# cliangyu/video-diffusion

Measured on AMD Instinct MI355X. Metric: denoise-steps/sec, higher is better.
Workload: dtype f32

## Files before the change

include/vd_amd.h:

```cpp
#ifndef VD_AMD_H
#define VD_AMD_H
#ifdef __cplusplus
extern "C" {
#endif

typedef struct vd_config {
    int image_size;
    int num_channels;
    int num_res_blocks;
    int num_heads;
    int T;
    int n_attention_ds;
    int attention_ds[8];
    int use_scale_shift_norm;
    int use_spatial_encoding;
    int use_frame_encoding;
    int enforce_position_invariance;
    int use_rpe_net;
    int allow_interactions_between_padding;
    float rp_alpha, rp_beta, rp_gamma;
    int time_embed_mult;
    int cond_emb_type;
    int learn_sigma;
} vd_config;
// ... 82 lines not shown
int vd_prior_bpd(vd_engine* e, int B, int T, const float* x_start, const float* latent_mask, float* out, void* stream);

int vd_score_windows(vd_engine* e, int B, int T, const float* x_start, const float* obs_mask, const float* latent_mask,
                     const float* kinda_marg_mask, const long long* frame_indices, const long long* t, int clip_denoised,
                     unsigned long long seed, const unsigned long long* item_offset, const float* noise, int suffix_skip,
                     double* mse_out, void* stream);
int vd_op_eps_mse(vd_engine* e, int B, int T, const float* x_start, const float* eps, const long long* t, int clip_denoised,
                  const float* latent_mask, unsigned long long seed, const unsigned long long* item_offset, const float* noise,
                  double* mse_out, void* stream);

int vd_window_begin(vd_engine* e, int B, int T, float* x, const float* obs_src, const float* obs_mask,
                    const float* latent_mask, const float* kinda_marg_mask, const long long* frame_indices,
                    int observed_frames, int sampler, int clip_denoised, float eta, unsigned long long seed,
                    unsigned long long offset, long long t_start, void* stream);
int vd_window_run(vd_engine* e, int n_steps, void* stream);
unsigned long long vd_window_generation(vd_engine* e);
int vd_window_graphs(vd_engine* e);

int vd_set_window_prefix_cache(vd_engine* e, int on);
int vd_window_prefix_frames(vd_engine* e);

int vd_set_window_suffix_skip(vd_engine* e, int on);
int vd_window_suffix_frames(vd_engine* e);

int vd_set_cfg_scale(vd_engine* e, float w);
float vd_cfg_scale(vd_engine* e);
int vd_op_cfg_combine(const float* out_c, const float* out_u, float w, long long n, float* out, void* stream);

int vd_set_guidance_rescale(vd_engine* e, float phi);
float vd_guidance_rescale(vd_engine* e);
int vd_set_dynamic_threshold(vd_engine* e, float p);
float vd_dynamic_threshold(vd_engine* e);
int vd_op_cfg_rescale(const float* out_c, const float* out_u, float w, const float* lat, int B, int T, long long frame_elems, float phi,
                      float* out, float* factor_out, void* stream);
int vd_op_dynamic_threshold(const float* x0, const float* lat, int B, int T, long long frame_elems, float p, float* out, float* s_out,
                            void* stream);

int vd_set_known_region(vd_engine* e, const float* known_src, const float* known_mask, const float* known_noise,
                        unsigned long long seed, unsigned long long offset);
int vd_known_region(vd_engine* e);
int vd_known_merge(vd_engine* e, int B, int T, long long frame_pixels, float* sample, const float* known_src, const float* known_mask,
                   const float* latent_mask, const long long* t, const float* known_noise, unsigned long long seed,
                   unsigned long long offset, void* stream);
int vd_set_jump_rows(vd_engine* e, int num_timesteps, const float* sqrt_alpha, const float* sqrt_beta);
int vd_q_jump(vd_engine* e, int B, int T, long long frame_pixels, const float* x, const float* latent_mask, const long long* t,
              const float* noise, unsigned long long seed, unsigned long long offset, float* out, void* stream);
// ... 157 lines not shown
```

video-diffusion_amd/_lib.py:

```python
import ctypes
import os
import subprocess

_HERE = os.path.dirname(os.path.abspath(__file__))
_CSRC = os.path.join(_HERE, "csrc")
SO_PATH = os.path.join(_HERE, "libvdamd.so")
SOURCES = ["igemm.hip", "conv_wino.hip", "conv_wino_r64.hip", "conv_wino_z128.hip", "gemm_frag.hip", "gemm_split.hip", "split_pack.hip", "norm.hip", "backward.hip", "attn_spatial.hip", "attn_temporal.hip", "attn_temporal_long.hip", "misc.hip", "guidance.hip", "known.hip", "measure.hip", "dps.hip", "engine.hip", "lpips.hip", "metrics.hip", "i3d.hip", "conv_cl.hip", "hallway.hip"]
HEADER = os.path.join(os.path.dirname(_HERE), "include", "vd_amd.h")
HEADERS = [os.path.join(_CSRC, "vd_common.h"), os.path.join(_CSRC, "wino_common.h"), os.path.join(_CSRC, "igemm_tile.h"), HEADER]
SOURCE_FLAGS = {"conv_wino_z128.hip": ["-mllvm", "-pragma-unroll-threshold=1000000"]}


def _toolchain():
    hipcc = os.environ.get("HIPCC", "/opt/rocm/bin/hipcc")
    flags = ["--offload-arch=gfx950", "-O3", "-std=c++17", "-fPIC", "-Wno-unused-value"] + \
        os.environ.get("VD_HIPCC_FLAGS", "").split()
    return hipcc, flags


def _sha(*parts):
    import hashlib
    h = hashlib.sha1()
    for p in parts:
        h.update(p if isinstance(p, bytes) else str(p).encode())
# ... 115 lines not shown
    "vd_pos_channels": (_I, [_P]),
    "vd_pos_resolution": (_I, [_P]),
    "vd_set_freqs": (_I, [_P, _P, _I, _P, _I]),
    "vd_set_schedule": (_I, [_P, _I, _P, _P, _F]),
    "vd_workspace_bytes": (_I, [_P, _I, _I, ctypes.POINTER(_L)]),
    "vd_unet_forward": (_I, [_P, _I, _I, _P, _P, _P, _P, _P, _P, _P, _I, _P, _P]),
    "vd_p_sample": (_I, [_P, _I, _I, _P, _P, _P, _P, _P, _P, _P, _I, _I, _P, _U, _U, _P, _P, _P, _P]),
    "vd_ddim_sample": (_I, [_P, _I, _I, _P, _P, _P, _P, _P, _P, _P, _I, _I, _F, _P, _U, _U, _P, _P, _P, _P]),
    "vd_ddim_reverse_sample": (_I, [_P, _I, _I, _P, _P, _P, _P, _P, _P, _P, _I, _I, _P, _P, _P, _P]),
    "vd_ddim_reverse_from_xstart": (_I, [_P, _I, _L, _P, _P, _P, _I, _P, _P, _P]),
    "vd_set_multistep_weights": (_I, [_P, _I, _P]),
    "vd_dpmpp_2m_sample": (_I, [_P, _I, _I, _P, _P, _P, _P, _P, _P, _P, _P, _I, _I, _P, _P, _P, _P]),
    "vd_dpmpp_2m_from_xstart": (_I, [_P, _I, _L, _P, _P, _P, _P, _I, _P, _P, _P]),
    "vd_p_mean_variance": (_I, [_P, _I, _I, _P, _P, _P, _P, _P, _P, _P, _I, _I, _P, _P, _P, _P]),
    "vd_vb_terms": (_I, [_P, _I, _I, _P, _P, _P, _P, _P, _I, _P, _P, _P, _P, _P, _P]),
    "vd_prior_bpd": (_I, [_P, _I, _I, _P, _P, _P, _P]),
    "vd_score_windows": (_I, [_P, _I, _I, _P, _P, _P, _P, _P, _P, _I, _U, _P, _P, _I, _P, _P]),
    "vd_op_eps_mse": (_I, [_P, _I, _I, _P, _P, _P, _I, _P, _U, _P, _P, _P, _P]),
    "vd_window_generation": (_U, [_P]),
    "vd_set_window_prefix_cache": (_I, [_P, _I]),
    "vd_window_prefix_frames": (_I, [_P]),
    "vd_set_window_suffix_skip": (_I, [_P, _I]),
    "vd_window_suffix_frames": (_I, [_P]),
    "vd_set_cfg_scale": (_I, [_P, _F]),
    "vd_cfg_scale": (_F, [_P]),
    "vd_op_cfg_combine": (_I, [_P, _P, _F, _L, _P, _P]),
    "vd_set_guidance_rescale": (_I, [_P, _F]),
    "vd_guidance_rescale": (_F, [_P]),
    "vd_set_dynamic_threshold": (_I, [_P, _F]),
    "vd_dynamic_threshold": (_F, [_P]),
    "vd_op_cfg_rescale": (_I, [_P, _P, _F, _P, _I, _I, _L, _F, _P, _P, _P]),
    "vd_op_dynamic_threshold": (_I, [_P, _P, _I, _I, _L, _F, _P, _P, _P]),
    "vd_set_known_region": (_I, [_P, _P, _P, _P, _U, _U]),
    "vd_known_region": (_I, [_P]),
    "vd_known_merge": (_I, [_P, _I, _I, _L, _P, _P, _P, _P, _P, _P, _U, _U, _P]),
    "vd_set_jump_rows": (_I, [_P, _I, _P, _P]),
    "vd_q_jump": (_I, [_P, _I, _I, _L, _P, _P, _P, _P, _U, _U, _P, _P]),
    "vd_window_jump": (_I, [_P, _I, _P]),
    "vd_set_measurement": (_I, [_P, _P, _I, _I]),
    "vd_measurement": (_I, [_P, _P, _P]),
    "vd_measurement_project": (_I, [_P, _I, _I, _I, _I, _P, _P, _P, _I, _I, _P]),
    "vd_window_begin": (_I, [_P, _I, _I, _P, _P, _P, _P, _P, _P, _I, _I, _I, _F, _U, _U, _L, _P]),
    "vd_window_run": (_I, [_P, _I, _P]),
    "vd_window_graphs": (_I, [_P]),
    "vd_posterior_update": (_I, [_P, _I, _I, _L, _P, _P, _P, _I, _F, _P, _U, _U, _P, _P, _P]),
    "vd_posterior_from_xstart": (_I, [_P, _I, _I, _L, _P, _P, _P, _I, _F, _P, _U, _U, _P, _P, _P, _P]),
# ... 71 lines not shown
    "vd_i3d_load_weight": (_I, [_P, ctypes.c_char_p, _P, _L]),
    "vd_i3d_max_frames": (_I, []),
    "vd_i3d_embed": (_I, [_P, _I, _I, _I, _I, _P, _P, _P]),
    "vd_op_conv3d_same": (_I, [_P, _P, _P, _I, _I, _I, _I, _I, _I, _I, _I, _I, _I, _I, _I, _P, _L, _P]),
    "vd_op_maxpool3d_same": (_I, [_P, _I, _I, _I, _I, _I, _I, _I, _I, _I, _I, _P, _P]),
    "vd_op_resize_bilinear_tf1": (_I, [_P, _I, _I, _I, _P, _P]),
    "vd_hallway_counts": (_I, [_I, _I, _I, _I, _I, _P, _I, _P, _P]),
    "vd_hallway_max_strip": (_I, []),
    "vd_op_green_mask": (_I, [_L, _P, _P, _P, _P]),
}

_lib = None


def lib():
    global _lib
    if _lib is None:
        path = os.environ.get("VD_LIB")
        if not path:
            build()
            path = SO_PATH
        L = ctypes.CDLL(path)
        for name, (res, args) in SIGNATURES.items():
            fn = getattr(L, name)
            fn.restype = res
            fn.argtypes = args
        if not os.environ.get("VD_LIB") and L.vd_source_sha().decode() != source_sha():
            raise RuntimeError(f"libvdamd.so was built from other sources ({L.vd_source_sha().decode()}) than the ones beside it "
                               f"({source_sha()}): rebuild (video_diffusion_amd._lib.build(force=True))")
        _lib = L
    return _lib


class VdError(RuntimeError):
    pass


def check(rc):
    if rc != 0:
        msg = lib().vd_last_error().decode(errors="replace")
        raise VdError(f"libvdamd error {rc}: {msg}")


def ptr(t):
    if t is None:
        return None
# ... 9 lines not shown
```

video-diffusion_amd/csrc/engine.hip:

```cpp
#include <cmath>
#include <cstring>
#include <unordered_map>
#include <vector>

#include "../../include/vd_amd.h"
#include "vd_common.h"

namespace vd {

thread_local std::string g_last_error;
void set_error(const std::string& msg) { g_last_error = msg; }

int launch_frame_t(const int64_t* fidx, int B, int T, int center, float* tv, hipStream_t s);

enum ParamKind { PK_RAW = 0, PK_CONV3, PK_STEM, PK_POSENC, PK_OUTCONV, PK_LINF, PK_CONV3W, PK_CONV3S,
                 PK_CONV3WU };

struct Param {
    std::string name;
    int nd = 0;
    long long shape[4] = {1, 1, 1, 1};
    size_t numel = 0;
    size_t packed = 0;
    size_t off = 0;
// ... 168 lines not shown
    std::vector<Param> params;
    std::unordered_map<std::string, int> pidx;
    std::vector<ResP> res;
    std::vector<AttnP> attn;
    std::vector<ConvP> convs;
    std::vector<std::vector<Layer>> input_blocks, output_blocks;
    std::vector<Layer> middle;
    int n_before_attn = 0, pos_res = 0, pos_ch = 0, final_ch = 0;
    int suf_blk = -2, suf_layer = -1;
    int p_posenc = -1, p_te0w, p_te0b, p_te2w, p_te2b, p_outgw, p_outgb, p_outw, p_outb;
    size_t film_w_off = 0, film_b_off = 0, te_w_off = 0, te_b_off = 0;
    int film_total = 0, te_total = 0;
    size_t packed_total = 0;
    float* wbuf = nullptr;
    bool wbuf_on_host = false;
    int put(void* dst, const void* src, size_t bytes) {
        if (wbuf_on_host) { std::memcpy(dst, src, bytes); return 0; }
        VD_HIP(hipMemcpy(dst, src, bytes, hipMemcpyHostToDevice));
        return 0;
    }
    struct RpeGroup { int C; std::vector<int> blocks; long long* d_hid = nullptr; long long* d_out = nullptr; };
    std::vector<RpeGroup> rpe_groups;
    std::vector<float*> rpe_R;
    int rpe_all(const float* te, const int64_t* fidx, int B, int T, hipStream_t st, Arena& ar);
    int rpe_tables();
    void rpe_group_blocks();
    float* d_freq_time = nullptr; int n_freq_time = 0;
    float* d_freq_frame = nullptr; int n_freq_frame = 0;
    float* d_tab = nullptr; int num_timesteps = 0;
    float* d_tmap = nullptr; float rescale = 1.f;
    float* d_w2m = nullptr;
    float* d_jump = nullptr;
    char* ws = nullptr; size_t ws_cap = 0;
    bool ws_suf = false;
    int ws_B = 0, ws_T = 0; size_t ws_tail = 0;
    std::unordered_map<long long, size_t> ws_peaks;
    static size_t tm_bytes(int B) { return ((size_t)B * sizeof(float) + 255) & ~(size_t)255; }
    size_t out_floats(int B, int T) const { return (size_t)B * T * (cfg.learn_sigma ? 6 : 3) * cfg.image_size * cfg.image_size; }
    size_t guid_off(int B, int T) const { return (tm_bytes(B) + 2 * out_floats(B, T) * sizeof(float) + 255) & ~(size_t)255; }
    size_t step_tail_bytes(int B, int T) const { return guid_off(B, T) + guidance_scratch_bytes(B); }
    float* step_tm() const { return reinterpret_cast<float*>(ws + ws_tail); }
    float* step_eps(int B) const { return reinterpret_cast<float*>(ws + ws_tail + tm_bytes(B)); }
    float* step_eps_u(int B, int T) const { return step_eps(B) + out_floats(B, T); }
    void* step_guid(int B, int T) const { return ws + ws_tail + guid_off(B, T); }
    Arena step_arena() const { Arena a; a.base = ws; a.cap = ws_tail; return a; }
    float* wbuf_bwd = nullptr; bool wbuf_bwd_on_host = false; size_t packed_bwd_total = 0;
    Tape* tape = nullptr;
// ... 73 lines not shown
        (void)hipDeviceSynchronize();
        for (auto& g : win_graphs) g.release();
        win_graphs.clear();
        win_cur = -1;
    }
    template <class Tp> int grow(Tp*& p, size_t& cap, size_t n, bool held_by_graphs) {
        if (n <= cap) return 0;
        if (held_by_graphs && p) { if (win_cur >= 0) win_lost = true; drop_window_graphs(); }
        if (p) VD_HIP(hipFree(p));
        p = nullptr; cap = 0;
        VD_HIP(hipMalloc(reinterpret_cast<void**>(&p), n * sizeof(Tp)));
        cap = n;
        return 0;
    }
    template <class DryRun> int grow_ws(long long key, size_t extra, DryRun dry_run, size_t* tail) {
        if (int rc = rpe_tables()) return rc;
        auto it = ws_peaks.find(key);
        if (it == ws_peaks.end()) {
            size_t peak = 0;
            if (int rc = dry_run(&peak)) return rc;
            it = ws_peaks.emplace(key, peak).first;
        }
        *tail = (it->second + 255) & ~(size_t)255;
        return grow(ws, ws_cap, *tail + extra, true);
    }

    const float* W(int p) const { return wbuf + params[p].off; }
    void set_w(vd::IgemmArgs& g, int p) const {
        const int k = params[p].kind;
        g.w = g.wfrag = g.wwino = nullptr;
        if (k == PK_CONV3W) { g.wwino = W(p); g.wsplit = split_math() ? 2 : 0; }
        else if (k == PK_CONV3WU) { g.wwino = W(p); g.wsplit = 2; g.ups_phase = 1; }
        else if (k == PK_CONV3S) { g.wfrag = W(p); g.wsplit = 1; }
        else if (k == PK_LINF) { g.wfrag = W(p); g.wsplit = split_math(); }
        else g.w = W(p);
    }

    int add(const std::string& name, std::initializer_list<long long> shape, int kind = PK_RAW) {
        Param p;
        p.name = name;
        p.nd = (int)shape.size();
        int i = 0;
        p.numel = 1;
        for (long long s : shape) { p.shape[i++] = s; p.numel *= (size_t)s; }
        p.kind = kind;
        p.packed = p.numel;
        const size_t O = (size_t)p.shape[0];
// ... 518 lines not shown
    if (!cfg.use_rpe_net || attn.empty() || !te_total) return 0;
    rpe_group_blocks();
    for (auto& g : rpe_groups) {
        if (g.d_hid) continue;
        const int nn = 3 * (int)g.blocks.size();
        std::vector<long long> th(3 * nn), to(2 * nn);
        for (size_t i = 0; i < g.blocks.size(); ++i) {
            const AttnP& a = attn[g.blocks[i]];
            const RpeP* rp[3] = {&a.rq, &a.rk, &a.rv};
            for (int k = 0; k < 3; ++k) {
                const int z = 3 * (int)i + k;
                th[3 * z] = rp[k]->te_off; th[3 * z + 1] = (long long)params[rp[k]->dw].off; th[3 * z + 2] = (long long)params[rp[k]->db].off;
                to[2 * z] = (long long)params[rp[k]->ow].off; to[2 * z + 1] = (long long)params[rp[k]->ob].off;
            }
        }
        VD_HIP(hipMalloc(reinterpret_cast<void**>(&g.d_hid), th.size() * sizeof(long long)));
        VD_HIP(hipMalloc(reinterpret_cast<void**>(&g.d_out), to.size() * sizeof(long long)));
        VD_HIP(hipMemcpy(g.d_hid, th.data(), th.size() * sizeof(long long), hipMemcpyHostToDevice));
        VD_HIP(hipMemcpy(g.d_out, to.data(), to.size() * sizeof(long long), hipMemcpyHostToDevice));
    }
    return 0;
}

int vd_engine::rpe_all(const float* te, const int64_t* fidx, int B, int T, hipStream_t st, Arena& ar) {
    rpe_R.clear();
    if (!cfg.use_rpe_net || attn.empty() || !te_total) return 0;
    rpe_group_blocks();
    const size_t rrows = (size_t)B * T * T;
    rpe_R.assign(3 * attn.size(), nullptr);
    int rc = 0;
    for (auto& g : rpe_groups) {
        const int nn = 3 * (int)g.blocks.size(), C = g.C;
        float* Rg = ar.get<float>((size_t)nn * rrows * C);
        for (size_t i = 0; i < g.blocks.size(); ++i)
            for (int k = 0; k < 3; ++k) rpe_R[3 * g.blocks[i] + k] = Rg + (3 * i + k) * rrows * C;
        const size_t mk = ar.mark();
        float* Eh = ar.get<float>((size_t)nn * rrows * C);
        ar.release(mk);
        if (ar.dry) continue;
        VD_REQUIRE(g.d_hid && g.d_out, "rpe_all: offset tables missing (ensure_ws builds them)");
        if ((rc = launch_rpe_hidden_tab(te, te_total, wbuf, g.d_hid, fidx, B, T, C, Eh, nn, rrows * C, st))) return rc;
        IgemmArgs q = linear_args((int)rrows, C, C);
        q.src0 = Eh; q.out = Rg;
        q.wfrag = wbuf + params[attn[g.blocks[0]].rq.ow].off; q.bias = wbuf + params[attn[g.blocks[0]].rq.ob].off;
        q.zcount = nn; q.zs_a = q.zs_out = (int)(rrows * C); q.ztab = g.d_out; q.zbase = wbuf;
        if ((rc = igemm_p(q, st))) return rc;
    }
    return 0;
}

int vd_engine::forward(const FwdIn& in, hipStream_t st, Arena& ar, const PrefixPlan* pp, const SuffixPlan* sp) {
    const int B = in.B, T = in.T, N = B * T, S = cfg.image_size, mc = cfg.num_channels;
    int rc;
    VD_REQUIRE(!pp || (!tape && !ar.dry && pp->store && n_before_attn > 0), "prefix plan: executor steps only");
    VD_REQUIRE(!sp || (!tape && sp->n > 0 && sp->n <= N && (ar.dry || sp->list)), "suffix plan: executor steps only, at least one frame");
    struct SelGuard { ~SelGuard() { g_sel_nfr = 0; } } sel_guard;
    const int Npre = pp ? pp->n : N;
    float* x8 = ar.get<float>((size_t)Npre * S * S * STEM_KPAD);
    float* tfr = ar.get<float>(N);
    float* amask = ar.get<float>(N);
    float* tsin = ar.get<float>((size_t)N * mc);
    float* e1 = ar.get<float>((size_t)N * E);
    float* emb = ar.get<float>((size_t)N * E);
    float* film = ar.get<float>((size_t)N * film_total);
    float* te = te_total ? ar.get<float>((size_t)N * te_total) : nullptr;
    float* ftv = cfg.use_frame_encoding ? ar.get<float>(N) : nullptr;
    float* femb = cfg.use_frame_encoding ? ar.get<float>((size_t)N * pos_ch) : nullptr;
    if (!ar.dry) {
        VD_REQUIRE(d_freq_time && n_freq_time == mc / 2, "vd_set_freqs not called (time frequencies)");
        AssembleArgs aa{in.x, in.obs_src, in.obs, in.lat, in.km, in.t_model, in.obs_mode, B, T, S, S, STEM_KPAD, cfg.cond_emb_type, x8, tfr, amask};
        if (pp) {
            AssembleArgs sc = aa; sc.scalars_only = 1;
            if ((rc = launch_assemble(sc, st))) return rc;
            aa.frame_list = pp->list; aa.n_list = pp->n;
        }
        if ((rc = launch_assemble(aa, st))) return rc;
        if ((rc = launch_sinus_embed(tfr, N, mc, d_freq_time, tsin, st))) return rc;
        if ((rc = linear(tsin, N, mc, E, W(p_te0w), W(p_te0b), 0, nullptr, e1, st))) return rc;
        if ((rc = linear(e1, N, E, E, W(p_te2w), W(p_te2b), 1, nullptr, emb, st))) return rc;
        if ((rc = linear(emb, N, E, film_total, wbuf + film_w_off, wbuf + film_b_off, 1, nullptr, film, st))) return rc;
        if (te_total && (rc = linear(emb, N, E, te_total, wbuf + te_w_off, wbuf + te_b_off, 0, nullptr, te, st))) return rc;
        if (cfg.use_frame_encoding) {
            VD_REQUIRE(d_freq_frame && n_freq_frame == pos_ch / 2, "vd_set_freqs not called (frame frequencies)");
            if ((rc = launch_frame_t(in.fidx, B, T, cfg.enforce_position_invariance, ftv, st))) return rc;
            if ((rc = launch_sinus_embed(ftv, N, pos_ch, d_freq_frame, femb, st))) return rc;
        }
    }
    rpe_R.clear();
    if (!(pp && pp->build_only) && (rc = rpe_all(te, in.fidx, B, T, st, ar))) return rc;
    attn_seq = 0;
    std::vector<Tens> hs;
    Tens h{x8, STEM_KPAD, S};
    int Nrun = Npre;
    const float* film_full = film;
    if (pp || ar.dry) {
        float* fc = ar.get<float>((size_t)std::max(pp ? Npre : N, 1) * film_total);
        if (pp) {
            if ((rc = launch_gather_rows(film_full, pp->list, Npre, film_total, fc, st))) return rc;
            film = fc;
        }
    }
    auto run = [&](const std::vector<Layer>& blk, Tens in0, const Tens* in1, Tens* outp, size_t l0 = 0, size_t l1 = ~(size_t)0) -> int {
        const int N = Nrun;
        Tens cur = in0;
        const Tens* second = in1;
        for (size_t li = l0; li < std::min(l1, blk.size()); ++li) {
            const Layer& L = blk[li];
            Tens nxt{};
            if (L.type == 1) {
                if ((rc = res_block(res[L.idx], cur, second, N, film, st, ar, &nxt))) return rc;
            } else if (L.type == 2) {
                if ((rc = attn_block(attn[L.idx], cur, B, T, in.fidx, amask, st, ar, &nxt))) return rc;
// ... 1162 lines not shown

int vd_op_dynamic_threshold(const float* x0, const float* lat, int B, int T, long long frame_elems, float p, float* out, float* s_out,
                            void* stream) {
    VD_REQUIRE(B > 0 && frame_elems > 0, "vd_op_dynamic_threshold: shape");
    OpScratch ws(stream);
    char* buf = nullptr;
    int rc = ws.get(&buf, guidance_scratch_bytes(B));
    if (rc) return rc;
    DynThreshArgs da{x0, nullptr, nullptr, nullptr, 0, lat, B, T, (long)frame_elems, p, out, s_out, nullptr, buf};
    return launch_dynamic_threshold(da, ws.st);
}

int vd_window_prefix_frames(vd_engine* e) {
    VD_REQUIRE(e, "null engine");
    return e->win_cur >= 0 && e->win_graphs[e->win_cur].store ? e->win_graphs[e->win_cur].n_inv : 0;
}

int vd_set_window_suffix_skip(vd_engine* e, int on) {
    VD_REQUIRE(e, "null engine");
    e->suffix_skip_on = on != 0;
    return 0;
}

int vd_window_suffix_frames(vd_engine* e) {
    VD_REQUIRE(e, "null engine");
    return e->win_cur >= 0 ? e->win_graphs[e->win_cur].n_suf : 0;
}

unsigned long long vd_window_generation(vd_engine* e) { return e ? e->win_gen : 0; }

int vd_window_run(vd_engine* e, int n_steps, void* stream) {
    VD_REQUIRE(e, "null engine");
    VD_REQUIRE(!e->win_lost, "window graphs invalidated (workspace growth or a new schedule since vd_window_begin): begin the window again");
    VD_REQUIRE(e->win_cur >= 0, "vd_window_begin first");
    const char* past = sampler_walks_up(e->win_graphs[e->win_cur].key.sampler) ? "more steps than the window has left (ddim_reverse_sample: t would pass num_timesteps - 1)"
                                                                  : "more steps than the window has left (t would pass 0)";
    VD_REQUIRE(n_steps >= 0 && n_steps <= e->win_left, past);
    hipStream_t st = static_cast<hipStream_t>(stream);
    for (int i = 0; i < n_steps; ++i) VD_HIP(hipGraphLaunch(e->win_graphs[e->win_cur].exec, st));
    e->win_left -= n_steps;
    return 0;
}

int vd_window_graphs(vd_engine* e) { return e ? (int)e->win_graphs.size() : -1; }

int vd_set_known_region(vd_engine* e, const float* known_src, const float* known_mask, const float* known_noise, unsigned long long seed,
// ... 688 lines not shown
```

video-diffusion_amd/csrc/gemm_split.hip:

```cpp
#include <cstring>
#include <vector>

#include "vd_common.h"

namespace vd {

typedef __bf16 bf16x4 __attribute__((ext_vector_type(4)));
typedef __bf16 bf16x8 __attribute__((ext_vector_type(8)));
typedef unsigned u32x4 __attribute__((ext_vector_type(4)));
typedef unsigned u32x2 __attribute__((ext_vector_type(2)));

template <bool F16>
__device__ __forceinline__ f32x16 mfma_piece(u32x4 a, u32x4 b, f32x16 c) {
    if constexpr (F16) return __builtin_amdgcn_mfma_f32_32x32x16_f16(__builtin_bit_cast(f16x8, a), __builtin_bit_cast(f16x8, b), c, 0, 0, 0);
    else return __builtin_amdgcn_mfma_f32_32x32x16_bf16(__builtin_bit_cast(bf16x8, a), __builtin_bit_cast(bf16x8, b), c, 0, 0, 0);
}

#ifndef VD_GS_SKIP
#define VD_GS_SKIP 0
#endif
#ifdef VD_GS_TIMING
__device__ unsigned long long g_gs_stamp[8];
#define GS_STAMP(i) do { if (threadIdx.x == 0 && blockIdx.x == gridDim.x / 2 && blockIdx.y == 0) {                        \
        __builtin_amdgcn_sched_barrier(0); g_gs_stamp[i] = __builtin_amdgcn_s_memrealtime(); __builtin_amdgcn_sched_barrier(0); } } while (0)
extern "C" int vd_debug_gs_stamps(unsigned long long* host_out) { return (int)hipMemcpyFromSymbol(host_out, HIP_SYMBOL(g_gs_stamp), sizeof(g_gs_stamp)); }
#else
#define GS_STAMP(i)
#endif
constexpr int SROW = 80;

template <bool F16>
__device__ __forceinline__ void split3(f32x4 v, u32x2& p1, u32x2& p2, u32x2& p3) {
    if constexpr (F16) {
        p1.x = f16_pack(v.x, v.y); p1.y = f16_pack(v.z, v.w);
        p2.x = f16_pack_scaled(f16_rem_lo(p1.x, v.x), f16_rem_hi(p1.x, v.y));
        p2.y = f16_pack_scaled(f16_rem_lo(p1.y, v.z), f16_rem_hi(p1.y, v.w));
        p3 = p2;
    } else {
        const bf16x4 q1 = __builtin_convertvector(v, bf16x4);
        f32x4 r = v - __builtin_convertvector(q1, f32x4);
        const bf16x4 q2 = __builtin_convertvector(r, bf16x4);
        r = r - __builtin_convertvector(q2, f32x4);
        const bf16x4 q3 = __builtin_convertvector(r, bf16x4);
        p1 = __builtin_bit_cast(u32x2, q1); p2 = __builtin_bit_cast(u32x2, q2); p3 = __builtin_bit_cast(u32x2, q3);
    }
}

template <int BM, int BN, bool ACT, bool CONV, bool F16 = true, bool SIDE = false>
__global__ __launch_bounds__(256, 2) void gemm_split_kernel(IgemmArgs a) {
    constexpr int MI = BM / 64, NI = BN / 64, AR = BM / 32;
    constexpr bool B2R = F16;
    constexpr int RING = NI >= 3 ? 2 : (BM == 64 && BN == 64) ? 6 : 3;
    constexpr int BP = B2R ? 2 : 3;
    constexpr int PF = BM == 64 ? 3 : 1;
    constexpr int NPL = F16 ? 2 : 3;
    constexpr int PLANE = BM * SROW, ABUF = NPL * PLANE;
    extern __shared__ __attribute__((aligned(16))) char smem_c[];
    const int tid = threadIdx.x, lane = tid & 63, wave = __builtin_amdgcn_readfirstlane(tid >> 6);
    GS_STAMP(0);
    const int wm = wave >> 1, wn = wave & 1;
    const int lr = lane & 31, lh = lane >> 5;
    int bxi = blockIdx.x, byi = blockIdx.y;
    if (gridDim.y > 1 && (gridDim.x & 7) == 0 && gridDim.x >= 128) {
        const unsigned lin = blockIdx.x + gridDim.x * blockIdx.y, xcd = lin & 7, loc = lin >> 3;
        byi = loc % gridDim.y;
        bxi = (loc / gridDim.y) * 8 + xcd;
    }
    const int m0 = bxi * BM, n0 = byi * BN;
    const int lgrp = tid >> 3, lrow = ((lgrp >> 1) & 3) + 8 * (lgrp >> 3) + 4 * (lgrp & 1), lq = tid & 7;
    const int cpt = a.Cin >> 5;
    const int nchunk = CONV ? 9 * cpt : cpt, ncoblk = a.Cout >> 5;
    const int C1 = a.Cin - a.C0;
    if (a.zcount > 1) {
        const int z = blockIdx.z;
        a.src0 += (size_t)z * a.zs_a; a.out += (size_t)z * a.zs_out;
        a.wfrag = a.zbase + a.ztab[2 * z];
        a.bias = a.zbase + a.ztab[2 * z + 1];
    }

    const auto asrc0 = __builtin_amdgcn_make_buffer_rsrc(const_cast<float*>(a.src0), 0,
                                                         (CONV ? a.nfr * a.Hs * a.Ws : a.M) * a.C0 * 4, 0x00020000);
    const auto asrc1 = __builtin_amdgcn_make_buffer_rsrc(const_cast<float*>(a.src1 ? a.src1 : a.src0), 0,
                                                         a.src1 ? a.M * C1 * 4 : 0, 0x00020000);
    unsigned ao0[AR], ao1[AR];
    int iy0[AR], ix0[AR];
#pragma unroll
    for (int j = 0; j < AR; ++j) {
        const unsigned row = (unsigned)min(m0 + lrow + 32 * j, a.M - 1);
        if constexpr (CONV) {
            const unsigned ox = row % (unsigned)a.Wo, t = row / (unsigned)a.Wo;
            const unsigned oy = t % (unsigned)a.Ho, n = t / (unsigned)a.Ho;
// ... 308 lines not shown
bool gemm_split_side_supported(const IgemmArgs& a) {
    return gemm_split_supported(a) && a.act == 0 && a.zcount <= 1 && gemm_split_tile_class(igemm_sel_M(a), a.Cout) == 0 &&
           a.side_hw > 0 && a.side_hw % 128 == 0 && a.M % a.side_hw == 0;
}

template <int BM, int BN, bool F16>
static int launch_gs_m(const IgemmArgs& a, hipStream_t s) {
    const size_t lds = (size_t)2 * (F16 ? 2 : 3) * BM * SROW;
    dim3 grid((a.M + BM - 1) / BM, (a.Cout + BN - 1) / BN, a.zcount > 1 ? a.zcount : 1);
    if (a.side) {
        if constexpr (BM == 128 && BN == 128) {
            VD_REQUIRE(gemm_split_side_supported(a) && a.sideA && a.sideB, "side output: plain 1x1 on the 128x128 tile, whole frames of a multiple of 128 rows");
            hipLaunchKernelGGL((gemm_split_kernel<128, 128, false, false, F16, true>), grid, dim3(256), lds, s, a);
            VD_HIP(hipGetLastError());
            return 0;
        } else {
            VD_REQUIRE(false, "side output: 128x128 tile only");
        }
    }
    if (a.ksz == 3) {
        if (a.act) hipLaunchKernelGGL((gemm_split_kernel<BM, BN, true, true, F16>), grid, dim3(256), lds, s, a);
        else hipLaunchKernelGGL((gemm_split_kernel<BM, BN, false, true, F16>), grid, dim3(256), lds, s, a);
    } else if (a.act) hipLaunchKernelGGL((gemm_split_kernel<BM, BN, true, false, F16>), grid, dim3(256), lds, s, a);
    else hipLaunchKernelGGL((gemm_split_kernel<BM, BN, false, false, F16>), grid, dim3(256), lds, s, a);
    VD_HIP(hipGetLastError());
    return 0;
}
template <int BM, int BN>
static int launch_gs(const IgemmArgs& a, hipStream_t s) {
    return f16_math() ? launch_gs_m<BM, BN, true>(a, s) : launch_gs_m<BM, BN, false>(a, s);
}

int gemm_split_tile_class(int M, int Cout) {
    const int base = igemm_tile_class(M, Cout);
    if (base != 0 || Cout % 192) return base;
    return (long)((M + 127) / 128) * (Cout / 192) >= 384 ? 4 : base;
}

int gemm_split_stats_rows(int M, int Cout) {
    const int c = gemm_split_tile_class(M, Cout);
    return c == 2 || c == 3 ? 32 : 64;
}

int launch_gemm_split(const IgemmArgs& a, int tile_class, hipStream_t s) {
    if (tile_class == 0) tile_class = gemm_split_tile_class(igemm_sel_M(a), a.Cout);
    if (a.stats) {
// ... 15 lines not shown
```

video-diffusion_amd/csrc/misc.hip:

```cpp
#include <algorithm>

#include "vd_common.h"

namespace vd {

__global__ __launch_bounds__(256) void assemble_kernel(AssembleArgs a) {
    const int n = a.frame_list ? a.frame_list[blockIdx.y] : blockIdx.y;
    const int HW = a.H * a.W;
    const float om = a.obs_mask[n], lm = a.lat_mask[n], km = a.km_mask[n];
    const float any = fminf(om + lm + km, 1.0f);
    const int Cs = a.cond_mode == 0 ? 5 : (a.cond_mode == 1 ? 6 : 3);
    if (blockIdx.x == 0 && threadIdx.x == 0 && !a.frame_list) {
        const float t = a.t_model[n / a.T];
        const float tobs = a.obs_t_mode == 0 ? 0.f : (a.obs_t_mode == 1 ? t : t - 1.f);
        float tf = t;
        if (a.cond_mode == 0) tf = tobs * om + t * (1.f - om);
        else if (a.cond_mode == 2) {
            bool any_obs = false;
            for (int k = 0; k < a.T; ++k) any_obs |= a.obs_mask[(n / a.T) * a.T + k] == 1.f;
            if (any_obs) tf = -1.f;
        }
        a.t_frames[n] = tf;
        a.amask[n] = any;
    }
// ... 110 lines not shown
    VD_HIP(hipGetLastError());
    return 0;
}

__global__ void frame_t_kernel(const int64_t* __restrict__ fidx, int T, int center, float* __restrict__ tv) {
    const int b = blockIdx.x;
    float mean = 0.f;
    if (center) {
        float s = 0.f;
        for (int t = 0; t < T; ++t) s += (float)fidx[b * T + t];
        mean = s / (float)T;
    }
    for (int t = threadIdx.x; t < T; t += blockDim.x) tv[b * T + t] = (float)fidx[b * T + t] - mean;
}

int launch_frame_t(const int64_t* fidx, int B, int T, int center, float* tv, hipStream_t s) {
    hipLaunchKernelGGL(frame_t_kernel, dim3(B), dim3(64), 0, s, fidx, T, center, tv);
    VD_HIP(hipGetLastError());
    return 0;
}

__global__ __launch_bounds__(256) void rpe_hidden_tab_kernel(const float* __restrict__ te, int te_ld, const float* __restrict__ wbase,
                                                             const long long* __restrict__ tab, const int64_t* __restrict__ fidx, int T, int C,
                                                             float* __restrict__ E, size_t zs_e) {
    __shared__ float feat[64][3];
    const long long* tz = tab + 3 * blockIdx.y;
    te += tz[0];
    const float* Wd = wbase + tz[1];
    const float* bd = wbase + tz[2];
    E += blockIdx.y * zs_e;
    const int bt = blockIdx.x, b = bt / T;
    for (int s0 = 0; s0 < T; s0 += 64) {
        const int ns = min(64, T - s0);
        __syncthreads();
        if ((int)threadIdx.x < ns) {
            const float d = (float)(fidx[bt] - fidx[b * T + s0 + threadIdx.x]);
            feat[threadIdx.x][0] = logf(1.0f + fmaxf(d, 0.f));
            feat[threadIdx.x][1] = logf(1.0f + fmaxf(-d, 0.f));
            feat[threadIdx.x][2] = d == 0.f ? 1.f : 0.f;
        }
        __syncthreads();
        for (int c = threadIdx.x; c < C; c += 256) {
            const float bc = bd[c], w0 = Wd[c * 3], w1 = Wd[c * 3 + 1], w2 = Wd[c * 3 + 2], tv = te[(size_t)bt * te_ld + c];
            for (int k = 0; k < ns; ++k) {
                const float lin = bc + feat[k][0] * w0 + feat[k][1] * w1 + feat[k][2] * w2;
                E[((size_t)bt * T + s0 + k) * C + c] = silu_f(tv + lin);
            }
        }
    }
}

int launch_rpe_hidden_tab(const float* te, int te_ld, const float* wbase, const long long* tab, const int64_t* fidx, int B, int T, int C,
                          float* E, int nz, size_t zs_e, hipStream_t s) {
    hipLaunchKernelGGL(rpe_hidden_tab_kernel, dim3(B * T, nz), dim3(256), 0, s, te, te_ld, wbase, tab, fidx, T, C, E, zs_e);
    VD_HIP(hipGetLastError());
    return 0;
}

__global__ __launch_bounds__(256) void rpe_table_kernel(const float* __restrict__ table, const int64_t* __restrict__ fidx,
                                                        int T, int C, float alpha, float beta, float gamma, double lg,
                                                        float* __restrict__ R) {
    const int row = blockIdx.x;
    const int s_ = row % T, bt = row / T, b = bt / T;
    const long long d = fidx[bt] - fidx[b * T + s_];
    long long id = d;
    const float ad = fabsf((float)d);
    if (ad > alpha) {
        double v = (double)alpha + log((double)ad / (double)alpha) / lg * ((double)beta - (double)alpha);
        const double r = rint(v);
        if (fabs(v - r) < 1e-6) v = r;
        v = fmin((double)beta, v);
        id = (long long)(int)v * (d > 0 ? 1 : -1);
    }
    const int nb = 2 * (int)beta + 1;
    if (id < 0) id += nb;
    for (int c = threadIdx.x; c < C; c += 256) R[(size_t)row * C + c] = table[(size_t)id * C + c];
}
// ... 606 lines not shown
```

video-diffusion_amd/csrc/vd_common.h:

```cpp
#pragma once
#include <hip/hip_runtime.h>
#include <cstdint>
#include <cstdio>
#include <string>

typedef float f32x4 __attribute__((ext_vector_type(4)));
typedef float f32x16 __attribute__((ext_vector_type(16)));

namespace vd {

constexpr int kMaxWindowFrames = 128;
constexpr int kMaxGuidedWindowFrames = 32;

void set_error(const std::string& msg);
extern thread_local std::string g_last_error;

#define VD_HIP(call)                                                                   \
    do {                                                                               \
        hipError_t e_ = (call);                                                        \
        if (e_ != hipSuccess) {                                                        \
            vd::set_error(std::string(#call) + ": " + hipGetErrorString(e_));          \
            return -2;                                                                 \
        }                                                                              \
    } while (0)
// ... 57 lines not shown
    int Ho, Wo;
    const float* w;
    const float* wfrag;
    const float* wwino;
    const float* bias;
    const float* affA;
    const float* affB;
    int act;
    const float* res;
    int res_ld;
    const float* fbias;
    int fbias_ld;
    float* out;
    int ldo;
    int Cout, M;
    double* stats;
    int stats_split;
    int stats_hw;
    int zcount, zs_a, zs_out;
    const long long* ztab = nullptr; const float* zbase = nullptr;
    int wsplit;
    float* ksplit_ws;
    size_t ksplit_ws_floats;
};

struct AttnSpatialArgs {
    const float* qkv;
    float* out;
    int nfr, L, C, heads;
    float scale;
};

struct AttnTemporalArgs {
    const float* qkv;
    const float* Rk;
    const float* Rq;
    const float* Rv;
    const float* mask;
    float* out;
    int B, T, HW, C, heads;
    int allow_pad;
    float scale;
};

enum ConvClGather {
    CG_QUAD,
// ... 146 lines not shown
                       hipStream_t s);

struct AssembleArgs {
    const float* x;
    const float* obs_src;
    const float* obs_mask, *lat_mask, *km_mask;
    const float* t_model;
    int obs_t_mode;
    int B, T, H, W, Kpad;
    int cond_mode;
    float* x_cols;
    float* t_frames;
    float* amask;
    const int* frame_list = nullptr;
    int n_list = 0;
    int scalars_only = 0;
};
int launch_assemble(const AssembleArgs& a, hipStream_t s);
int launch_gather_rows(const float* src, const int* list, int n, size_t row_floats, float* dst, hipStream_t s);
int launch_scatter_rows(const float* src, const int* list, int n, size_t row_floats, float* dst, hipStream_t s);
int launch_scatter_stats(const double* src, int split, int C, const int* list, int n, double* dst, hipStream_t s);
int launch_sinus_embed(const float* t, int n, int dim, const float* freqs, float* out, hipStream_t s);
int launch_rpe_hidden_tab(const float* te, int te_ld, const float* wbase, const long long* tab, const int64_t* fidx, int B, int T, int C,
                          float* E, int nz, size_t zs_e, hipStream_t s);
int launch_rpe_table(const float* table, const int64_t* fidx, int B, int T, int C, float alpha, float beta,
                     float gamma, float* R, hipStream_t s);
int launch_posenc_add(const float* x, const float* P, const float* femb, int nfr, int HW, int C, float* y,
                      hipStream_t s);
int launch_frame_t(const int64_t* fidx, int B, int T, int center, float* tv, hipStream_t s);
int launch_out_conv(const float* x, const float* affA, const float* affB, const float* w, const float* bias, int nfr,
                    int H, int W, int C, int Cout, float* out_nchw, hipStream_t s);

bool head_gemm_supported(int HW, int C, int ldt);
int launch_head_gemm(const float* h, const float* affA, const float* affB, const float* Wt, int nfr, int HW, int C, int ldt, float* T, hipStream_t s);
int launch_out_gather(const float* T, const float* bias, int nfr, int H, int W, int ldt, int Cout, float* out_nchw, hipStream_t s);

enum Sampler { SAMPLER_P = 0, SAMPLER_DDIM = 1, SAMPLER_DDIM_REVERSE = 2, SAMPLER_DPMPP_2M = 3 };
inline bool sampler_valid(int s) { return s >= SAMPLER_P && s <= SAMPLER_DPMPP_2M; }
inline bool sampler_walks_up(int s) { return s == SAMPLER_DDIM_REVERSE; }
inline bool sampler_draws_noise(int s) { return s == SAMPLER_P || s == SAMPLER_DDIM; }
inline bool sampler_has_history(int s) { return s == SAMPLER_DPMPP_2M; }
inline const char* sampler_name(int s) {
    return s == SAMPLER_P ? "p_sample" : s == SAMPLER_DDIM ? "ddim_sample" : s == SAMPLER_DDIM_REVERSE ? "ddim_reverse_sample" : "dpmpp_2m_sample";
}
struct SamplerPassArgs {
    int sampler;
    const float* x;
// ... 252 lines not shown
```

Baseline: 50.53.

## Deduplicate RPE network evaluation across batch items with identical frame times and indices

Adds a device-side map that finds batch items whose frame times and frame indices match an earlier item. The RPE hidden-feature kernel and the RPE linear GEMM skip tiles belonging to duplicate items, and a replicate kernel then copies the representative item's RPE tables to the duplicates. This targets redundant relative-position-embedding computation when batch items share the same timestep and frame layout. In exchange it adds a small single-block kernel and a copy pass, rotates GEMM tile order to spread the live work, and falls back to full work when items differ.

```diff
diff --git a/include/vd_amd.h b/include/vd_amd.h
--- a/include/vd_amd.h
+++ b/include/vd_amd.h
@@ -128,6 +128,10 @@
 
 int vd_set_window_suffix_skip(vd_engine* e, int on);
 int vd_window_suffix_frames(vd_engine* e);
+
+int vd_set_rpe_dedup(vd_engine* e, int on);
+int vd_rpe_dedup(vd_engine* e);
+int vd_rpe_live_items(vd_engine* e, int* out, int cap);
 
 int vd_set_cfg_scale(vd_engine* e, float w);
 float vd_cfg_scale(vd_engine* e);
diff --git a/video-diffusion_amd/_lib.py b/video-diffusion_amd/_lib.py
--- a/video-diffusion_amd/_lib.py
+++ b/video-diffusion_amd/_lib.py
@@ -161,6 +161,9 @@
     "vd_window_prefix_frames": (_I, [_P]),
     "vd_set_window_suffix_skip": (_I, [_P, _I]),
     "vd_window_suffix_frames": (_I, [_P]),
+    "vd_set_rpe_dedup": (_I, [_P, _I]),
+    "vd_rpe_dedup": (_I, [_P]),
+    "vd_rpe_live_items": (_I, [_P, _P, _I]),
     "vd_set_cfg_scale": (_I, [_P, _F]),
     "vd_cfg_scale": (_F, [_P]),
     "vd_op_cfg_combine": (_I, [_P, _P, _F, _L, _P, _P]),
@@ -278,6 +281,9 @@
             path = SO_PATH
         L = ctypes.CDLL(path)
         for name, (res, args) in SIGNATURES.items():
+            fn = getattr(L, name, None)
+            if fn is None and os.environ.get("VD_LIB"):
+                continue
             fn = getattr(L, name)
             fn.restype = res
             fn.argtypes = args
diff --git a/video-diffusion_amd/csrc/engine.hip b/video-diffusion_amd/csrc/engine.hip
--- a/video-diffusion_amd/csrc/engine.hip
+++ b/video-diffusion_amd/csrc/engine.hip
@@ -214,7 +214,9 @@
     struct RpeGroup { int C; std::vector<int> blocks; long long* d_hid = nullptr; long long* d_out = nullptr; };
     std::vector<RpeGroup> rpe_groups;
     std::vector<float*> rpe_R;
-    int rpe_all(const float* te, const int64_t* fidx, int B, int T, hipStream_t st, Arena& ar);
+    bool rpe_dedup_on = true;
+    const int* rpe_live_last = nullptr; int rpe_live_B = 0;
+    int rpe_all(const float* te, const float* tfr, const int64_t* fidx, int B, int T, int* rep, int* live, hipStream_t st, Arena& ar);
     int rpe_tables();
     void rpe_group_blocks();
     float* d_freq_time = nullptr; int n_freq_time = 0;
@@ -334,7 +336,10 @@
             it = ws_peaks.emplace(key, peak).first;
         }
         *tail = (it->second + 255) & ~(size_t)255;
-        return grow(ws, ws_cap, *tail + extra, true);
+        const char* ws_was = ws;
+        const int rc = grow(ws, ws_cap, *tail + extra, true);
+        if (ws != ws_was) { rpe_live_last = nullptr; rpe_live_B = 0; }
+        return rc;
     }
 
     const float* W(int p) const { return wbuf + params[p].off; }
@@ -899,13 +904,21 @@
     return 0;
 }
 
-int vd_engine::rpe_all(const float* te, const int64_t* fidx, int B, int T, hipStream_t st, Arena& ar) {
+int vd_engine::rpe_all(const float* te, const float* tfr, const int64_t* fidx, int B, int T, int* rep, int* live, hipStream_t st, Arena& ar) {
     rpe_R.clear();
     if (!cfg.use_rpe_net || attn.empty() || !te_total) return 0;
     rpe_group_blocks();
     const size_t rrows = (size_t)B * T * T;
     rpe_R.assign(3 * attn.size(), nullptr);
     int rc = 0;
+    const bool dedup = rpe_dedup_on && rep && live;
+    if (!ar.dry) {
+        rpe_live_last = nullptr; rpe_live_B = 0;
+        if (dedup) {
+            if ((rc = launch_rpe_rep_map(tfr, fidx, B, T, rep, live, st))) return rc;
+            rpe_live_last = live; rpe_live_B = B;
+        }
+    }
     for (auto& g : rpe_groups) {
         const int nn = 3 * (int)g.blocks.size(), C = g.C;
         float* Rg = ar.get<float>((size_t)nn * rrows * C);
@@ -916,12 +929,14 @@
         ar.release(mk);
         if (ar.dry) continue;
         VD_REQUIRE(g.d_hid && g.d_out, "rpe_all: offset tables missing (ensure_ws builds them)");
-        if ((rc = launch_rpe_hidden_tab(te, te_total, wbuf, g.d_hid, fidx, B, T, C, Eh, nn, rrows * C, st))) return rc;
+        if ((rc = launch_rpe_hidden_tab(te, te_total, wbuf, g.d_hid, fidx, B, T, C, Eh, nn, rrows * C, st, dedup ? live : nullptr))) return rc;
         IgemmArgs q = linear_args((int)rrows, C, C);
         q.src0 = Eh; q.out = Rg;
         q.wfrag = wbuf + params[attn[g.blocks[0]].rq.ow].off; q.bias = wbuf + params[attn[g.blocks[0]].rq.ob].off;
         q.zcount = nn; q.zs_a = q.zs_out = (int)(rrows * C); q.ztab = g.d_out; q.zbase = wbuf;
+        if (dedup) { q.row_live = live; q.row_live_rows = T * T; }
         if ((rc = igemm_p(q, st))) return rc;
+        if (dedup && (rc = launch_rpe_replicate(Rg, rep, B, T, C, nn, rrows * C, st))) return rc;
     }
     return 0;
 }
@@ -936,6 +951,8 @@
     float* x8 = ar.get<float>((size_t)Npre * S * S * STEM_KPAD);
     float* tfr = ar.get<float>(N);
     float* amask = ar.get<float>(N);
+    int* rpe_rep = ar.get<int>(B);
+    int* rpe_live = ar.get<int>(B);
     float* tsin = ar.get<float>((size_t)N * mc);
     float* e1 = ar.get<float>((size_t)N * E);
     float* emb = ar.get<float>((size_t)N * E);
@@ -964,7 +981,7 @@
         }
     }
     rpe_R.clear();
-    if (!(pp && pp->build_only) && (rc = rpe_all(te, in.fidx, B, T, st, ar))) return rc;
+    if (!(pp && pp->build_only) && (rc = rpe_all(te, tfr, in.fidx, B, T, rpe_rep, rpe_live, st, ar))) return rc;
     attn_seq = 0;
     std::vector<Tens> hs;
     Tens h{x8, STEM_KPAD, S};
@@ -2173,6 +2190,24 @@
     return 0;
 }
 
+int vd_set_rpe_dedup(vd_engine* e, int on) {
+    VD_REQUIRE(e, "null engine");
+    if ((on != 0) != e->rpe_dedup_on) { if (e->win_cur >= 0) e->win_lost = true; e->drop_window_graphs(); }
+    e->rpe_dedup_on = on != 0;
+    return 0;
+}
+
+int vd_rpe_dedup(vd_engine* e) { return e && e->rpe_dedup_on ? 1 : 0; }
+
+int vd_rpe_live_items(vd_engine* e, int* out, int cap) {
+    VD_REQUIRE(e && out && cap >= 0, "vd_rpe_live_items: arguments");
+    if (!e->rpe_live_last) return 0;
+    VD_HIP(hipDeviceSynchronize());
+    const int n = std::min(cap, e->rpe_live_B);
+    VD_HIP(hipMemcpy(out, e->rpe_live_last, (size_t)n * sizeof(int), hipMemcpyDeviceToHost));
+    return e->rpe_live_B;
+}
+
 int vd_window_suffix_frames(vd_engine* e) {
     VD_REQUIRE(e, "null engine");
     return e->win_cur >= 0 ? e->win_graphs[e->win_cur].n_suf : 0;
diff --git a/video-diffusion_amd/csrc/gemm_split.hip b/video-diffusion_amd/csrc/gemm_split.hip
--- a/video-diffusion_amd/csrc/gemm_split.hip
+++ b/video-diffusion_amd/csrc/gemm_split.hip
@@ -46,7 +46,7 @@
     }
 }
 
-template <int BM, int BN, bool ACT, bool CONV, bool F16 = true, bool SIDE = false>
+template <int BM, int BN, bool ACT, bool CONV, bool F16 = true, bool SIDE = false, bool LIVE = false>
 __global__ __launch_bounds__(256, 2) void gemm_split_kernel(IgemmArgs a) {
     constexpr int MI = BM / 64, NI = BN / 64, AR = BM / 32;
     constexpr bool B2R = F16;
@@ -66,7 +66,15 @@
         byi = loc % gridDim.y;
         bxi = (loc / gridDim.y) * 8 + xcd;
     }
+    static_assert(!LIVE || (!ACT && !CONV && !SIDE), "row_live: the plain 1x1 only");
+    if constexpr (LIVE) bxi = (int)(((unsigned)bxi + (byi + blockIdx.z) * (unsigned)max(a.row_live_rows / BM, 1)) % gridDim.x);
     const int m0 = bxi * BM, n0 = byi * BN;
+    if constexpr (LIVE) {
+        const int mlast = min(m0 + BM, a.M) - 1;
+        int any = 0;
+        for (int i = m0 / a.row_live_rows; i * a.row_live_rows <= mlast; ++i) any |= a.row_live[i];
+        if (!any) return;
+    }
     const int lgrp = tid >> 3, lrow = ((lgrp >> 1) & 3) + 8 * (lgrp >> 3) + 4 * (lgrp & 1), lq = tid & 7;
     const int cpt = a.Cin >> 5;
     const int nchunk = CONV ? 9 * cpt : cpt, ncoblk = a.Cout >> 5;
@@ -421,6 +429,10 @@
         if (a.act) hipLaunchKernelGGL((gemm_split_kernel<BM, BN, true, true, F16>), grid, dim3(256), lds, s, a);
         else hipLaunchKernelGGL((gemm_split_kernel<BM, BN, false, true, F16>), grid, dim3(256), lds, s, a);
     } else if (a.act) hipLaunchKernelGGL((gemm_split_kernel<BM, BN, true, false, F16>), grid, dim3(256), lds, s, a);
+    else if (a.row_live) {
+        VD_REQUIRE(a.row_live_rows > 0, "row_live: rows per item");
+        hipLaunchKernelGGL((gemm_split_kernel<BM, BN, false, false, F16, false, true>), grid, dim3(256), lds, s, a);
+    }
     else hipLaunchKernelGGL((gemm_split_kernel<BM, BN, false, false, F16>), grid, dim3(256), lds, s, a);
     VD_HIP(hipGetLastError());
     return 0;
diff --git a/video-diffusion_amd/csrc/misc.hip b/video-diffusion_amd/csrc/misc.hip
--- a/video-diffusion_amd/csrc/misc.hip
+++ b/video-diffusion_amd/csrc/misc.hip
@@ -156,8 +156,9 @@
 
 __global__ __launch_bounds__(256) void rpe_hidden_tab_kernel(const float* __restrict__ te, int te_ld, const float* __restrict__ wbase,
                                                              const long long* __restrict__ tab, const int64_t* __restrict__ fidx, int T, int C,
-                                                             float* __restrict__ E, size_t zs_e) {
+                                                             float* __restrict__ E, size_t zs_e, const int* __restrict__ live) {
     __shared__ float feat[64][3];
+    if (live && !live[blockIdx.x / T]) return;
     const long long* tz = tab + 3 * blockIdx.y;
     te += tz[0];
     const float* Wd = wbase + tz[1];
@@ -185,8 +186,69 @@
 }
 
 int launch_rpe_hidden_tab(const float* te, int te_ld, const float* wbase, const long long* tab, const int64_t* fidx, int B, int T, int C,
-                          float* E, int nz, size_t zs_e, hipStream_t s) {
-    hipLaunchKernelGGL(rpe_hidden_tab_kernel, dim3(B * T, nz), dim3(256), 0, s, te, te_ld, wbase, tab, fidx, T, C, E, zs_e);
+                          float* E, int nz, size_t zs_e, hipStream_t s, const int* live) {
+    hipLaunchKernelGGL(rpe_hidden_tab_kernel, dim3(B * T, nz), dim3(256), 0, s, te, te_ld, wbase, tab, fidx, T, C, E, zs_e, live);
+    VD_HIP(hipGetLastError());
+    return 0;
+}
+
+constexpr int REP_MAX_B = 1024;
+__global__ __launch_bounds__(256) void rpe_rep_map_kernel(const float* __restrict__ tfr, const int64_t* __restrict__ fidx, int B, int T,
+                                                          int* __restrict__ rep, int* __restrict__ live) {
+    __shared__ int rs[REP_MAX_B];
+    const unsigned* tb = reinterpret_cast<const unsigned*>(tfr);
+    auto same = [&](int b, int c) {
+        bool eq = true;
+        for (int t = 0; t < T; ++t)
+            eq &= (tb[(size_t)c * T + t] == tb[(size_t)b * T + t]) & (fidx[(size_t)c * T + t] == fidx[(size_t)b * T + t]);
+        return eq;
+    };
+    if (B > REP_MAX_B) {
+        for (int b = threadIdx.x; b < B; b += blockDim.x) {
+            int r = b;
+            for (int c = 0; c < b && r == b; ++c) if (same(b, c)) r = c;
+            rep[b] = r;
+            live[b] = r == b ? 1 : 0;
+        }
+        return;
+    }
+    for (int b = threadIdx.x; b < B; b += blockDim.x) rs[b] = b;
+    __syncthreads();
+    for (int p = threadIdx.x; p < B * B; p += blockDim.x) {
+        const int b = p / B, c = p - b * B;
+        if (c < b && same(b, c)) atomicMin(&rs[b], c);
+    }
+    __syncthreads();
+    for (int b = threadIdx.x; b < B; b += blockDim.x) { rep[b] = rs[b]; live[b] = rs[b] == b ? 1 : 0; }
+}
+
+int launch_rpe_rep_map(const float* tfr, const int64_t* fidx, int B, int T, int* rep, int* live, hipStream_t s) {
+    hipLaunchKernelGGL(rpe_rep_map_kernel, dim3(1), dim3(256), 0, s, tfr, fidx, B, T, rep, live);
+    VD_HIP(hipGetLastError());
+    return 0;
+}
+
+constexpr int REPL_QUADS = 4;
+__global__ __launch_bounds__(256) void rpe_replicate_kernel(float* __restrict__ R, const int* __restrict__ rep, size_t item4, size_t zs4) {
+    const int b = blockIdx.y, r = rep[b];
+    if (r == b) return;
+    f32x4* base = reinterpret_cast<f32x4*>(R) + blockIdx.z * zs4;
+    const f32x4* src = base + (size_t)r * item4;
+    f32x4* dst = base + (size_t)b * item4;
+    const size_t i0 = (size_t)blockIdx.x * (256 * REPL_QUADS) + threadIdx.x;
+    f32x4 v[REPL_QUADS];
+#pragma unroll
+    for (int k = 0; k < REPL_QUADS; ++k) if (i0 + k * 256 < item4) v[k] = src[i0 + k * 256];
+#pragma unroll
+    for (int k = 0; k < REPL_QUADS; ++k) if (i0 + k * 256 < item4) dst[i0 + k * 256] = v[k];
+}
+
+int launch_rpe_replicate(float* R, const int* rep, int B, int T, int C, int nz, size_t zs_r, hipStream_t s) {
+    const size_t item = (size_t)T * T * C;
+    VD_REQUIRE(item % 4 == 0 && zs_r % 4 == 0 && zs_r >= (size_t)B * item && ((uintptr_t)R & 15) == 0, "rpe_replicate: 16-byte quads");
+    VD_REQUIRE(B <= 65535 && nz <= 65535, "rpe_replicate: grid");
+    const size_t per = 256 * REPL_QUADS;
+    hipLaunchKernelGGL(rpe_replicate_kernel, dim3((unsigned)((item / 4 + per - 1) / per), B, nz), dim3(256), 0, s, R, rep, item / 4, zs_r / 4);
     VD_HIP(hipGetLastError());
     return 0;
 }
diff --git a/video-diffusion_amd/csrc/vd_common.h b/video-diffusion_amd/csrc/vd_common.h
--- a/video-diffusion_amd/csrc/vd_common.h
+++ b/video-diffusion_amd/csrc/vd_common.h
@@ -103,6 +103,8 @@
     int wsplit;
     float* ksplit_ws;
     size_t ksplit_ws_floats;
+    const int* row_live = nullptr;
+    int row_live_rows = 0;
 };
 
 struct AttnSpatialArgs {
@@ -295,7 +297,9 @@
 int launch_scatter_stats(const double* src, int split, int C, const int* list, int n, double* dst, hipStream_t s);
 int launch_sinus_embed(const float* t, int n, int dim, const float* freqs, float* out, hipStream_t s);
 int launch_rpe_hidden_tab(const float* te, int te_ld, const float* wbase, const long long* tab, const int64_t* fidx, int B, int T, int C,
-                          float* E, int nz, size_t zs_e, hipStream_t s);
+                          float* E, int nz, size_t zs_e, hipStream_t s, const int* live = nullptr);
+int launch_rpe_rep_map(const float* tfr, const int64_t* fidx, int B, int T, int* rep, int* live, hipStream_t s);
+int launch_rpe_replicate(float* R, const int* rep, int B, int T, int C, int nz, size_t zs_r, hipStream_t s);
 int launch_rpe_table(const float* table, const int64_t* fidx, int B, int T, int C, float alpha, float beta,
                      float gamma, float* R, hipStream_t s);
 int launch_posenc_add(const float* x, const float* P, const float* femb, int nfr, int HW, int C, float* y,
```

New measurement: 50.77 (median of 6 runs). No clear change (+0.5%).
